# raguilar011095/planet_heightmap_generation

Hardware: AMD Instinct MI355X
Metric: Mcells·iter/s, terrain-post erosion stack (higher is better)
Workload: dtype f64

## Files before the change

planet_heightmap_generation_amd/csrc/basin.hip:

```cpp
#include <hip/hip_runtime.h>

#include <string>

#include "device.h"

namespace wo {

namespace {

constexpr int32_t WO_RANGE_NONE = 0x7f7f7f7f;
#ifndef WO_BASIN_RANGE_SLOTS
#define WO_BASIN_RANGE_SLOTS 256
#endif
constexpr int WO_BASIN_RANGE = WO_BASIN_RANGE_SLOTS;
constexpr int WO_BASIN_KEY_BITS = 16;
constexpr int WO_BASIN_CHASE_CAP = 1 << 16;

__device__ inline int32_t basin_root(int32_t* J, int32_t s) {
    auto ld = [&](int32_t x) { return __atomic_load_n(&J[x], __ATOMIC_RELAXED); };
    int32_t j = ld(s), tort = j;
    int power = 1, lam = 0;
    for (int it = 0; it < WO_BASIN_CHASE_CAP; ++it) {
        const int32_t jj = ld(j);
        if (jj == j) return j;
        if (jj == tort) {
            int32_t m = jj, y = ld(jj);
            for (int k = 0; k < WO_BASIN_CHASE_CAP && y != jj; ++k) {
                const int32_t yy = ld(y);
                if (yy == y) return y;
                m = y < m ? y : m;
                y = yy;
            }
            __atomic_store_n(&J[m], m, __ATOMIC_RELAXED);
            return m;
        }
        if (++lam == power) { tort = jj; power <<= 1; lam = 0; }
        j = jj;
    }
    return j;
}

__global__ __launch_bounds__(WO_BLOCK) void k_basin_jump(const int32_t* __restrict__ slotCell, int32_t* J, int32_t L, int32_t shift, uint32_t* __restrict__ keyOfCell) {
    for (int32_t s = blockIdx.x * blockDim.x + threadIdx.x; s < L; s += gridDim.x * blockDim.x) {
        const int32_t j = basin_root(J, s);
        __atomic_store_n(&J[s], j, __ATOMIC_RELAXED);
        keyOfCell[slotCell ? slotCell[s] : s] = (uint32_t)j >> shift;
    }
}
__global__ __launch_bounds__(WO_BLOCK) void k_basin_keys(const int32_t* __restrict__ land, const uint32_t* __restrict__ keyOfCell, int32_t L,
                                                          uint32_t* __restrict__ keys, int32_t* __restrict__ vals, int32_t scramble, int32_t* rangeStart, int32_t nRangeWords) {
    for (int32_t i = blockIdx.x * blockDim.x + threadIdx.x; i < nRangeWords; i += gridDim.x * blockDim.x) rangeStart[i] = WO_RANGE_NONE;
    if (blockIdx.x == 0 && threadIdx.x == 0) rangeStart[nRangeWords] = 0;
    for (int32_t i = blockIdx.x * blockDim.x + threadIdx.x; i < L; i += gridDim.x * blockDim.x) {
        const int32_t c = land[L - 1 - i];
        keys[i] = (scramble && c % 3 == 0) ? (keyOfCell[c] ^ 1u) : keyOfCell[c];
        vals[i] = c;
    }
}

__global__ __launch_bounds__(WO_BLOCK) void k_basin_slots(const int32_t* __restrict__ order, const uint32_t* __restrict__ keys, int32_t* __restrict__ slotOf, int32_t L,
                                                           int32_t* rangeStart, int32_t rangeT) {
    for (int32_t q = blockIdx.x * blockDim.x + threadIdx.x; q < L; q += gridDim.x * blockDim.x) {
        if (slotOf) slotOf[order[q]] = q;
        if (q == 0 || keys[q] != keys[q - 1]) atomicMin(&rangeStart[q / rangeT], q);
    }
}

#ifndef WO_LONG_RANGE_SLOTS
#define WO_LONG_RANGE_SLOTS 2048
#endif
#ifndef WO_LONG_LIST
#define WO_LONG_LIST 2048
#endif
constexpr int32_t WO_LONG_RANGE = WO_LONG_RANGE_SLOTS, WO_LONG_MAX = WO_LONG_LIST;
__device__ inline int32_t range_end(const int32_t* __restrict__ rangeStart, int32_t k, int32_t nRanges, int32_t L) {
    for (int32_t j = k + 1; j < nRanges; ++j) { const int32_t v = rangeStart[j]; if (v != WO_RANGE_NONE) return v; }
    return L;
}
__global__ __launch_bounds__(WO_BLOCK) void k_basin_long(const int32_t* __restrict__ rangeStart, int32_t nRanges, int32_t L, int32_t* big, uint8_t* __restrict__ flag) {
    for (int32_t k = blockIdx.x * blockDim.x + threadIdx.x; k < nRanges; k += gridDim.x * blockDim.x) {
        const int32_t S = rangeStart[k];
        uint8_t f = 0;
        if (S != WO_RANGE_NONE && range_end(rangeStart, k, nRanges, L) - S >= WO_LONG_RANGE) {
            const int32_t at = atomicAdd(&big[0], 1);
            if (at < WO_LONG_MAX) { big[1 + at] = k; f = 1; }
        }
        flag[k] = f;
    }
}
__device__ inline bool block_range(const int32_t* __restrict__ rangeStart, int32_t nRanges, int32_t L, const int32_t* __restrict__ big, const uint8_t* __restrict__ flag, int32_t& S, int32_t& E) {
    int32_t k;
    if (big) {
        if ((int32_t)blockIdx.x < WO_LONG_MAX) { const int32_t n = big[0] < WO_LONG_MAX ? big[0] : WO_LONG_MAX; if ((int32_t)blockIdx.x >= n) return false; k = big[1 + blockIdx.x]; }
        else { k = (int32_t)blockIdx.x - WO_LONG_MAX; if (flag[k]) return false; }
    } else k = (int32_t)blockIdx.x;
    S = rangeStart[k];
    if (S == WO_RANGE_NONE) return false;
    E = range_end(rangeStart, k, nRanges, L);
// ... 174 lines not shown
        if (lane == 0) { s_passes[wave] = myPasses; s_readyPasses[wave] = myReady; }
        if (tid == 0) { s_clk[0] = cWait; s_clk[1] = cTurn; s_clk[2] = myPasses; s_clk[3] = cRest; }
        __syncthreads();
        if (tid == 0) {
            const unsigned long long c = (unsigned long long)(clock64() - cStart);
            const unsigned long long packed = (c << 24) | (unsigned long long)(s_maxLevel & 0xffffff);
            const unsigned long long old = atomicMax(&stats[0], packed);
            if (packed > old) {
                stats[1] = (unsigned long long)(E - S);
                unsigned long long mp = 0, mr = 0;
                for (int w = 0; w < NW; ++w) { mp = s_passes[w] > mp ? s_passes[w] : mp; mr = s_readyPasses[w] > mr ? s_readyPasses[w] : mr; }
                stats[2] = mp; stats[3] = mr; stats[4] = s_clk[0]; stats[5] = s_clk[1]; stats[6] = s_clk[2]; stats[7] = s_clk[3];
            }
        }
    }
}

}

void basin_alloc(wo_planet* p) {
    const int32_t N = p->N;
    hipStream_t s = cur_stream(p);
    if (!p->d_basinJ) {
        WO_HIP(hipMalloc((void**)&p->d_basinJ, (size_t)N * 4));
        WO_HIP(hipMalloc((void**)&p->d_basinSlot, (size_t)N * 4));
        WO_HIP(hipMalloc((void**)&p->d_basinKey, (size_t)N * 4));
        WO_HIP(hipMalloc((void**)&p->d_basinVals[0], (size_t)N * 4)); WO_HIP(hipMalloc((void**)&p->d_basinVals[1], (size_t)N * 4));
        WO_HIP(hipMalloc((void**)&p->d_basinRange, ((size_t)N / 64 + 8 + WO_LONG_MAX) * 4));
        WO_HIP(hipMalloc((void**)&p->d_basinLong, (size_t)N / 64 + 8));
        WO_HIP(hipMemsetAsync(p->d_basinSlot, 0xff, (size_t)N * 4, s));
    }
}

void basin_layout(wo_planet* p, bool slotIdentity) {
    const int32_t L = p->L;
    basin_alloc(p);
    int bitsL = 1;
    while (((int64_t)1 << bitsL) < (int64_t)L) ++bitsL;
    const int shift = bitsL > WO_BASIN_KEY_BITS ? bitsL - WO_BASIN_KEY_BITS : 0;
    const int grid = blocks_for(L, 1 << 16);
    launch(p, FAM_BASIN, k_basin_jump, grid, WO_BLOCK, slotIdentity ? (const int32_t*)nullptr : (const int32_t*)p->d_patchOrder, p->d_basinJ, L, (int32_t)shift, p->d_basinKey);
    const int rangeT = WO_BASIN_RANGE;
    const int nRanges = (int)(((int64_t)L + rangeT - 1) / rangeT);
    launch(p, FAM_BASIN, k_basin_keys, grid, WO_BLOCK, (const int32_t*)p->d_land[p->landCur], (const uint32_t*)p->d_basinKey, L, p->d_keys[0], p->d_basinVals[0],
           (int32_t)(p->opt.basinScramble ? 1 : 0), p->d_basinRange, (int32_t)(nRanges + 1));
    uint32_t* const kb[2] = {p->d_keys[0], p->d_keys[1]};
    int32_t* const vb[2] = {p->d_basinVals[0], p->d_basinVals[1]};
    const int sorted = radix_sort_pairs(p, FAM_BASIN_SORT, kb, vb, L, 0, 16 , p->d_basinSlot, radix_scratch(p, 1), p->N, p->rsFlip[1]);
    launch(p, FAM_BASIN, k_basin_slots, blocks_for(L, 4096), WO_BLOCK, (const int32_t*)p->d_basinVals[sorted], (const uint32_t*)p->d_keys[sorted], (int32_t*)nullptr, L, p->d_basinRange, (int32_t)rangeT);
    launch(p, FAM_BASIN, k_basin_long, blocks_for(nRanges), WO_BLOCK, (const int32_t*)p->d_basinRange, (int32_t)nRanges, L, p->d_basinRange + nRanges + 1, p->d_basinLong);
}

void basin_solve_launch(wo_planet* p, const Fields& F, int32_t launchTag, int32_t* totalPending) {
    const int nRanges = (int)(((int64_t)p->L + WO_BASIN_RANGE - 1) / WO_BASIN_RANGE);
    ++p->basinLaunches;
    const int32_t* big = (const int32_t*)(p->d_basinRange + nRanges + 1);
    const uint8_t* flag = (const uint8_t*)p->d_basinLong;
    const int grid = nRanges + WO_LONG_MAX;
    launch(p, FAM_SOLVE_BASIN, k_solve_flowing<2, false>, grid, 128, F, p->L, (const int32_t*)p->d_basinRange, (int32_t)nRanges, launchTag, p->d_patchPending, totalPending, big, flag, (unsigned long long*)nullptr);
}

void basin_free(wo_planet* p) {
    if (p->d_basinJ) (void)hipFree(p->d_basinJ);
    if (p->d_basinSlot) (void)hipFree(p->d_basinSlot);
    if (p->d_basinKey) (void)hipFree(p->d_basinKey);
    for (auto& v : p->d_basinVals) { if (v) (void)hipFree(v); v = nullptr; }
    if (p->d_basinRange) (void)hipFree(p->d_basinRange);
    if (p->d_basinLong) (void)hipFree(p->d_basinLong);
    p->d_basinLong = nullptr;
    p->d_basinJ = nullptr; p->d_basinSlot = nullptr; p->d_basinKey = nullptr; p->d_basinRange = nullptr;
}

}
```

planet_heightmap_generation_amd/csrc/device.h:

```cpp
#pragma once
#include <hip/hip_runtime.h>

#include <cstdint>
#include <cstdio>
#include <map>
#include <string>
#include <vector>

#include "host_util.h"

#include "erode_ops.h"
#include "flood_ops.h"
#include "wo_internal.h"

namespace wo {

struct HipError { std::string msg; };

#define WO_HIP(call)                                                                                   \
    do {                                                                                               \
        hipError_t e_ = (call);                                                                        \
        if (e_ != hipSuccess)                                                                          \
            throw ::wo::HipError{std::string(#call) + " -> " + hipGetErrorString(e_) + " (" + __FILE__ + ":" + \
                                 std::to_string(__LINE__) + ")"};                                      \
// ... 82 lines not shown
    wo::FloodExchange floodX;
    void* floodLink = nullptr; void (*floodLinkFree)(void*) = nullptr;
    wo_flood_gpu fgpu;

    int32_t *d_off = nullptr, *d_adj = nullptr;
    float *d_dist = nullptr, *d_xyz = nullptr;
    float *d_e = nullptr, *d_e2 = nullptr, *d_hot = nullptr, *d_orig = nullptr;
    uint8_t *d_ocean = nullptr, *d_coast = nullptr;
    int64_t mirrorMaskVersion = -1;
    uint8_t* d_oceanKnown = nullptr; int32_t* d_maskDiff = nullptr; bool oceanKnownValid = false;
    bool hot_valid = false;
    float* d_savedE = nullptr; uint8_t* d_savedOcean = nullptr; bool saved = false;
    uint8_t* d_tables = nullptr;
    bool scratch = false;
    bool landIdentity = false;
    int64_t floodPrefixMirror = -1, floodPrefixStatic = -1;
    bool floodPrefixOk = false;
    int32_t *d_landIdx = nullptr, *d_land[2] = {nullptr, nullptr}, *d_rank = nullptr;
    int32_t* d_landInit = nullptr; int64_t oceanVersion = 0, landListsOcean = -1; bool landListsMirror = false; int32_t landListsL = -1;
    uint32_t* d_keys[2] = {nullptr, nullptr};
    float *d_cellDist = nullptr, *d_flow = nullptr;
    wo::SolveTask* d_task = nullptr; wo::SolveOut* d_out = nullptr; int32_t *d_haloSend = nullptr, *d_haloRecv = nullptr; float *d_haloBuf = nullptr, *h_haloBuf = nullptr; int32_t nHaloSend = 0, nHaloRecv = 0;
    int32_t* d_flowCnt = nullptr; wo::TargetRank* d_tr = nullptr; wo::EventList* d_ev = nullptr; float* d_me = nullptr;
    int32_t *d_carveSlot = nullptr, *d_carveDeps = nullptr, *d_carveDepCnt = nullptr, *d_carveDepPos = nullptr; uint32_t* d_rs[2] = {nullptr, nullptr}; int rsFlip[2] = {0, 0};    wo::CarveRec* d_carveRecs = nullptr; wo::CarveExpect* d_carveExpect = nullptr; unsigned long long* d_carveG = nullptr;    int32_t* d_carveSlotDone = nullptr; int64_t carveCap = 0;
    unsigned long long* d_accCnt = nullptr;
    int32_t *d_ftLr = nullptr, *d_ftParent = nullptr, *d_ftExtCnt = nullptr; uint32_t* d_ftInflow = nullptr; unsigned long long* d_ftRootAcc = nullptr;
    int32_t *d_jump = nullptr, *d_nj = nullptr;
    int32_t* d_doneAt = nullptr;
    double* d_totalExcess = nullptr;
    float *d_glac = nullptr, *d_iceFlow = nullptr;
    int32_t *d_iceTarget = nullptr, *d_arank = nullptr;
    uint8_t* d_iceUp = nullptr;
    int32_t *d_patchOrder = nullptr, *d_slotOf = nullptr, *d_patchPending = nullptr, *d_patchTotals = nullptr, *d_patchBlk = nullptr; int64_t patchVersion = -1; bool patchMirror = false; int32_t numPatches = 0; int64_t lastPatchLaunches = 1; int64_t solveCalls = 0;
    hipStream_t side = nullptr; hipEvent_t evFork = nullptr, evJoin = nullptr; bool onSide = false;
    uint32_t* d_basinKey = nullptr; int32_t* d_basinVals[2] = {nullptr, nullptr}; int32_t *d_basinJ = nullptr, *d_basinSlot = nullptr, *d_basinRange = nullptr; uint8_t* d_basinLong = nullptr; int64_t basinLaunches = 0; wo::Affine* d_affine[2] = {nullptr, nullptr};    int64_t solvePassSerial = 0;
    int32_t* h_patchTotals = nullptr;
    int32_t *d_listA = nullptr, *d_listB = nullptr, *d_counters = nullptr;
    void* d_sortTemp = nullptr; size_t sortTempBytes = 0;
    int landCur = 0;
    int32_t L = 0;

    struct Import {
        uint8_t* img = nullptr; int64_t imgCap = 0;
        int32_t* label = nullptr;
        uint8_t* flags = nullptr;
        int32_t* lists = nullptr;
        uint8_t* seedOcean = nullptr;
        int32_t* blockCounts = nullptr;
        int32_t* totals = nullptr; int32_t* h_totals = nullptr;
    } imp;

    struct wo_wind_block* wind = nullptr;
    struct wo_ocean_block* ocean = nullptr;

    struct Mirror {
        bool built = false, active = false;
        int32_t *perm = nullptr, *inv = nullptr, *off = nullptr, *adj = nullptr;
        float *dist = nullptr, *xyz = nullptr, *e = nullptr, *e2 = nullptr, *hot = nullptr;
        uint8_t *ocean = nullptr, *coast = nullptr;
        wo::hvec<int32_t> h_perm, h_morton;
        wo::hvec<uint8_t> h_mask;
        int64_t version = 0;
        int32_t *o_off = nullptr, *o_adj = nullptr; float *o_dist = nullptr, *o_xyz = nullptr, *o_e = nullptr, *o_e2 = nullptr;
        uint8_t *o_ocean = nullptr, *o_coast = nullptr;
    } mirror;

    hipEvent_t evStart = nullptr, evStop = nullptr;
// ... 20 lines not shown

template <class... KArgs, class... Args>
inline void launch(wo_planet* p, int fam, void (*kernel)(KArgs...), int grid, int block, Args... args) {
    hipStream_t s = cur_stream(p);
    if (p->profiling) {
        hipEvent_t a = profile_event(p), b = profile_event(p);
        WO_HIP(hipEventRecord(a, s));
        hipLaunchKernelGGL(kernel, dim3(grid), dim3(block), 0, s, args...);
        WO_HIP(hipGetLastError());
        WO_HIP(hipEventRecord(b, s));
        p->pending.push_back({fam, a, b});
        if (p->pending.size() >= 4096) profile_resolve(p);
    } else {
        hipLaunchKernelGGL(kernel, dim3(grid), dim3(block), 0, s, args...);
        WO_HIP(hipGetLastError());
    }
}

template <class... KArgs, class... Args>
inline void launch_shmem(wo_planet* p, int fam, void (*kernel)(KArgs...), int grid, int block, size_t shmem, Args... args) {
    hipStream_t s = p->ctx->stream;
    hipEvent_t a = nullptr, b = nullptr;
    if (p->profiling) { a = profile_event(p); b = profile_event(p); WO_HIP(hipEventRecord(a, s)); }
    if (shmem > (size_t)(64 << 10)) WO_HIP(hipFuncSetAttribute(reinterpret_cast<const void*>(kernel), hipFuncAttributeMaxDynamicSharedMemorySize, (int)shmem));
    hipLaunchKernelGGL(kernel, dim3(grid), dim3(block), shmem, s, args...);
    WO_HIP(hipGetLastError());
    if (p->profiling) { WO_HIP(hipEventRecord(b, s)); p->pending.push_back({fam, a, b}); if (p->pending.size() >= 4096) profile_resolve(p); }
}

void sort_land_by_elevation(wo_planet* p);
size_t sort_temp_bytes(int32_t n);
void rank_from_land(wo_planet* p);
size_t radix_scratch_words(int32_t nMax);
int radix_sort_pairs(wo_planet* p, int family, uint32_t* const keys[2], int32_t* const vals[2], int32_t n, int beginBit, int endBit, int32_t* posOut,
                     uint32_t* scratch, int32_t nMax, int& flip);
uint32_t* radix_scratch(wo_planet* p, int which);
void select_active_by_rank(wo_planet* p, const int32_t* arank, int32_t* out, int32_t* outCount);
void basin_alloc(wo_planet* p);
void basin_layout(wo_planet* p, bool slotIdentity);
void basin_solve_launch(wo_planet* p, const Fields& F, int32_t launchTag, int32_t* totalPending);
void basin_free(wo_planet* p);
void import_free(wo_planet* p);
void wind_free(wo_planet* p);
void ocean_free(wo_planet* p);
bool check_planet(wo_planet* p, const char* fn);
float* smooth_field_resident(wo_planet* p, float* a, float* b, int32_t passes);

}
```

planet_heightmap_generation_amd/csrc/planet.hip:

```cpp
#include <hip/hip_runtime.h>

#include <algorithm>
#include <atomic>
#include <chrono>
#include <cmath>
#include <cstring>

#include "../../include/worogen.h"
#include "device.h"
#include "elevation_host.h"
#include "elevation_kernels.h"
#include "kernels_impl.h"
#include "flood_kernels.h"
#include "elevation_bfs.h"
#include "noise.h"

namespace wo {

const char* const kFamilyNames[FAM_COUNT] = {
    "coast_flags", "smooth_elevation", "sharpen_ridges", "soil_creep", "warp_terrain", "noise_eval", "synthetic_terrain",
    "ocean_from_elevation", "sort_keys", "sort_radix", "rank_scatter", "receivers", "flow_climb",
    "flow_final", "solve_setup", "solve_round", "solve_final", "thermal_excess", "thermal_apply",
    "glac_index", "ice_receivers", "ice_round", "carve_setup", "carve_round", "moraine_fjord", "glacial_blend", "solve_patch", "elev_collisions", "elev_uplift_fused", "plate_grid", "plate_project", "smooth_field", "flood_eval", "flood_apply", "flood_misc", "climate_sweeps", "basin_layout", "basin_sort", "solve_basin", "flow_tiles", "misc", "event_pair_empty", "event_pair_noop_kernel", "event_pair_two_noop_kernels"};

// ... 458 lines not shown
        const int32_t N = p->N;
        launch(p, FAM_MISC, k_mirror_gather_f32, blocks_for(N, 4096), WO_BLOCK, (const float*)p->d_e, (const int32_t*)M.perm, M.e, N);
        launch(p, FAM_MISC, k_mirror_gather_u8, blocks_for(N, 4096), WO_BLOCK, (const uint8_t*)p->d_ocean, (const int32_t*)M.perm, M.ocean, N);
        M.o_off = p->d_off; M.o_adj = p->d_adj; M.o_dist = p->d_dist; M.o_xyz = p->d_xyz; M.o_e = p->d_e; M.o_e2 = p->d_e2; M.o_ocean = p->d_ocean; M.o_coast = p->d_coast;
        point_at_mirror(M.e, M.e2);
        M.active = on = true;
    }
    void suspend() {
        if (!on) return;
        auto& M = p->mirror;
        launch(p, FAM_MISC, k_mirror_scatter_f32, blocks_for(p->N, 4096), WO_BLOCK, (const float*)p->d_e, (const int32_t*)M.perm, M.o_e, p->N);
        cur = p->d_e; cur2 = p->d_e2;
        point_at_planet();
    }
    void resume() {
        if (!on) return;
        auto& M = p->mirror;
        launch(p, FAM_MISC, k_mirror_gather_f32, blocks_for(p->N, 4096), WO_BLOCK, (const float*)M.o_e, (const int32_t*)M.perm, cur, p->N);
        point_at_mirror(cur, cur2);
    }
    void finish() {
        if (!on) return;
        suspend();
        p->mirror.active = on = false;
    }
    ~MirrorScope() { if (on) { point_at_planet(); p->mirror.active = false; } }
};

static void ensure_side_stream(wo_planet* p) {
    if (p->side) return;
    int prLeast = 0, prGreatest = 0;
    WO_HIP(hipDeviceGetStreamPriorityRange(&prLeast, &prGreatest));
    WO_HIP(hipStreamCreateWithPriority(&p->side, hipStreamNonBlocking, prGreatest));
    WO_HIP(hipEventCreateWithFlags(&p->evFork, hipEventDisableTiming)); WO_HIP(hipEventCreateWithFlags(&p->evJoin, hipEventDisableTiming));
}

struct RedoWithChecks {};

struct ErodeCall {
    wo_planet* p;
    int32_t hIters; double K, m, dt; int32_t tIters; double talus, kThermal; int32_t gIters; double gStrength; bool checkEveryPass;
    int32_t total, midIter; double gCarve, gConv, gDep, gFjord;
    int gridN, gridL = 0;
    StageClock clk; MirrorScope mir; FloodRun floodRun;
    int64_t sorts = 0, maxSolve = 0, patchLaunches = 0, basinPasses = 0, basinLeftoverPasses = 0, iceRounds = 0, carveRounds = 0, carveActive = 0, carveFlowLeft = 0;
    double floodHostMs = 0;
    ErodeCall(wo_planet* pl, int32_t h, double K_, double m_, double dt_, int32_t t, double talus_, double kT, int32_t g, double gs, bool check)
        : p(pl), hIters(h), K(K_), m(m_), dt(dt_), tIters(t), talus(talus_), kThermal(kT), gIters(std::max(g, 0)), gStrength(gs != gs ? 0 : gs),
          checkEveryPass(check), total(std::max(hIters, std::max(tIters, gIters))), midIter((int32_t)std::floor(total * 0.75 + 0.5)),
          gridN(xcd_grid(pl->N)), clk(pl), mir(pl) {
        const double gScale = gIters > 0 ? 1.0 / gIters : 0;
        gCarve = 0.02 * gScale; gConv = 0.01 * gScale; gDep = 0.005 * gScale; gFjord = 0.015 * gScale;
    }
    void stats(bool mirrored) const {
        p->erodeStats = {{"land_cells", (double)p->L}, {"mirror_layout", mirrored ? 1.0 : 0.0}, {"iterations", (double)total}, {"sorts", (double)sorts},
                         {"solve_launches_max_per_pass", (double)maxSolve}, {"solve_patch_launches_total", (double)patchLaunches},
                         {"solve_basin_passes", (double)basinPasses}, {"solve_basin_passes_with_leftovers", (double)basinLeftoverPasses},
                         {"flow_two_level", (p->d_ftLr && p->landIdentity && hIters > 0) ? 1.0 : 0.0}, {"ice_rounds_total", (double)iceRounds},
                         {"carve_rounds_total", (double)carveRounds}, {"carve_active_total", (double)carveActive}, {"carve_flow_launches_with_leftovers", (double)carveFlowLeft}, {"solve_check_every_pass", checkEveryPass ? 1.0 : 0.0}, {"calls_run_again_with_checks", (double)p->redoCalls}, {"flood_stage_ms", floodHostMs},
                         {"flood_device_pass1_ms", floodRun.deviceMs}, {"flood_device_rounds", (double)floodRun.rounds}, {"flood_device_epochs", (double)floodRun.epochs},
                         {"flood_device_evaluations", (double)floodRun.evals}, {"flood_equal_key_decisions", (double)floodRun.ties}, {"flood_pass1_on_host", (floodRun.usedDevice && !floodRun.fellBack) ? 0.0 : 1.0},
                         {"flood_host_calls", (double)floodRun.host.calls}, {"flood_host_serial_pass1", (double)floodRun.host.serialPass1}, {"flood_host_tie_groups", (double)floodRun.host.tieGroups}, {"flood_host_contested", (double)floodRun.host.contested},
                         {"flood_host_open_parents", (double)floodRun.host.openParents}, {"flood_host_unresolved", (double)floodRun.host.unresolved},
                         {"flood_host_path_redo", (double)floodRun.host.pathRedo}, {"flood_host_replays", (double)floodRun.host.replays}, {"flood_host_replayed_landmasses", (double)floodRun.host.replayedLandmasses}, {"flood_host_pass1_ms", floodRun.host.pass1Ms},
                         {"flood_host_pass23_ms", floodRun.host.pass23Ms},
                         {"relaxed_sort_every", (double)p->opt.relaxedSortEvery}, {"relaxed_full", p->opt.relaxedFull ? 1.0 : 0.0}, {"flood_exchange_calls", (double)p->floodX.calls}, {"flood_exchange_gathers", (double)p->floodX.gathers}, {"flood_exchange_whole_planet_floods", (double)p->floodX.globalFloods}, {"flood_exchange_received", (double)p->floodX.received}};
    }
// ... 165 lines not shown
    c.clk.begin("glacial");
    Fields F = p->fields();
    ice_flow(c, F);
    launch(p, FAM_CARVE_SETUP, k_carve_setup_cells, c.gridN, WO_BLOCK, F);
    select_active_by_rank(p, F.arank, p->d_listB, p->d_counters + 3);
    const int32_t active = read_count(p, p->d_counters + 3);
    c.carveActive += active; ensure_carve_capacity(p, active);
    F.carveDeps = p->d_carveDeps; F.carveDepCnt = p->d_carveDepCnt; F.carveDepPos = p->d_carveDepPos;
    if (active > 0) c.carveRounds += carve_launches(c, F, active);
    launch(p, FAM_MORAINE, k_moraine_fjord, c.gridN, WO_BLOCK, F, c.gDep, c.gFjord);
    c.clk.end();
}
static FlowTiles flow_tiles_buffers(wo_planet* p) {
    const size_t N = (size_t)p->N;
    if (!p->d_ftLr) {
        p->d_ftLr = dalloc<int32_t>(N); p->d_ftParent = dalloc<int32_t>(N); p->d_ftExtCnt = dalloc<int32_t>(N); p->d_ftInflow = dalloc<uint32_t>(N); p->d_ftRootAcc = dalloc<unsigned long long>(N);
        WO_HIP(hipMemsetAsync(p->d_ftInflow, 0, N * 4, p->ctx->stream)); WO_HIP(hipMemsetAsync(p->d_ftExtCnt, 0, N * 4, p->ctx->stream));
    }
    FlowTiles FT{};
    FT.lr = p->d_ftLr; FT.parent = p->d_ftParent; FT.rootAcc = p->d_ftRootAcc; FT.inflow = p->d_ftInflow; FT.extCnt = p->d_ftExtCnt;
    return FT;
}
static int flow_tile_count(int32_t L) { return (int)(((int64_t)L + FT_CELLS - 1) / FT_CELLS); }
static void erode_receivers(ErodeCall& c, const Fields& F, const FlowTiles& FT, int32_t* donorCnt, bool basin, bool slotIdentity, bool tilesBeforeFork) {
    wo_planet* p = c.p; hipStream_t s = p->ctx->stream;
    Fields Fr = F; if (basin) Fr.basinJ = p->d_basinJ;
    c.clk.begin("receivers");
    launch(p, FAM_RECEIVERS, k_receivers_flow_init, c.gridL, WO_BLOCK, Fr, donorCnt);
    c.clk.end();
    if (!basin) return;
    ensure_side_stream(p);
    if (tilesBeforeFork) {
        launch(p, FAM_FLOW_TILES, k_flow_tiles<false>, flow_tile_count(p->L), FT_THREADS, F, FT);
        launch(p, FAM_FLOW_TILES, k_flow_root_links, blocks_for(p->L, 4096), WO_BLOCK, F, FT);
    }
    WO_HIP(hipEventRecord(p->evFork, s));
    WO_HIP(hipStreamWaitEvent(p->side, p->evFork, 0));
    p->onSide = true;
    try { basin_layout(p, slotIdentity); } catch (...) { p->onSide = false; throw; }
    p->onSide = false;
    WO_HIP(hipEventRecord(p->evJoin, p->side));
}
static void erode_flow(ErodeCall& c, const Fields& F, const FlowTiles& FT, int32_t* donorCnt, bool flowTiles, bool tilesBeforeFork, bool clearOut) {
    wo_planet* p = c.p;
    c.clk.begin("flow");
    if (flowTiles) {
        const int tiles = flow_tile_count(p->L);
        if (!tilesBeforeFork) {
            launch(p, FAM_FLOW_TILES, k_flow_tiles<false>, tiles, FT_THREADS, F, FT);
            launch(p, FAM_FLOW_TILES, k_flow_root_links, blocks_for(p->L, 4096), WO_BLOCK, F, FT);
        }
        launch(p, FAM_FLOW_TILES, k_flow_root_climb, blocks_for(p->L, 4096), WO_BLOCK, F, FT);
        launch(p, FAM_FLOW_TILES, k_flow_tiles<true>, tiles, FT_THREADS, F, FT);
    } else
        launch(p, FAM_FLOW_SNAP, k_flow_climb, c.gridL, WO_BLOCK, F, (const int32_t*)p->d_flowCnt, (int32_t)0x7fffffff);
    Fields Ff = F;
    if (p->opt.relaxedFull) Ff.ev = nullptr;
    launch(p, FAM_FLOW_FINAL, k_flow_final, c.gridL, WO_BLOCK, Ff, donorCnt, clearOut ? p->d_out : (SolveOut*)nullptr);
    c.clk.end();
}
static void erode_solve_basin(ErodeCall& c, Fields F, int32_t iter) {
    wo_planet* p = c.p; hipStream_t s = p->ctx->stream;
    WO_HIP(hipStreamWaitEvent(s, p->evJoin, 0));
    F.slotOf = p->d_basinSlot; F.solveLean = 1;
    const bool unchecked = !c.checkEveryPass; F.solveFinals = unchecked ? 1 : 0;
    launch(p, FAM_SOLVE_SETUP, k_solve_setup_batched<true>, c.gridL, WO_BLOCK, F, p->d_patchPending, (int32_t)p->numPatches, p->d_patchTotals, (int32_t)WO_PATCH_TOTAL_SLOTS);
    int32_t passTag = 1;
    if (unchecked) {
        if (p->solvePassSerial >= 0x3ff00000) { WO_HIP(hipMemsetAsync(p->d_out, 0, (size_t)p->N * sizeof(SolveOut), s)); p->solvePassSerial = 0; }
        passTag = (1 << 20) + (int32_t)(++p->solvePassSerial);
    }
    const int64_t r = run_solve_patches(p, F, c.K, c.m, c.dt, unchecked, passTag);
    ++c.basinPasses; if (r > 1) ++c.basinLeftoverPasses;
    c.patchLaunches += r; c.maxSolve = std::max(c.maxSolve, r);
    if (!unchecked) launch(p, FAM_SOLVE_FINAL, k_solve_final, c.gridL, WO_BLOCK, F, p->d_e2, (iter < c.tIters) ? p->d_me : (float*)nullptr);
}
static void erode_solve_affine(ErodeCall& c, const Fields& F) {
    wo_planet* p = c.p;
    if (!p->d_affine[0]) { p->d_affine[0] = dalloc<Affine>((size_t)p->N); p->d_affine[1] = dalloc<Affine>((size_t)p->N); }
    launch(p, FAM_SOLVE_SETUP, k_affine_init, c.gridL, WO_BLOCK, F, p->d_affine[0]);
    int cur = 0;
    for (int q = 0; q < 12; ++q, cur ^= 1) launch(p, FAM_SOLVE_ROUND, k_affine_jump, c.gridL, WO_BLOCK, F, (const Affine*)p->d_affine[cur], p->d_affine[cur ^ 1]);
    launch(p, FAM_SOLVE_FINAL, k_affine_apply, c.gridL, WO_BLOCK, F, (const Affine*)p->d_affine[cur], p->d_e2);
}
static void hydraulic_step(ErodeCall& c, int32_t iter) {
    wo_planet* p = c.p;
    Fields F = p->fields();
    F.solveK = c.K; F.solveM = c.m; F.solveDt = c.dt;
    const bool basin = !p->opt.relaxedFull;
    const bool slotIdentity = c.mir.on && p->mirror.h_mask.size() == (size_t)p->N;
    if (basin) { basin_alloc(p); F.basinMslot = slotIdentity ? nullptr : p->d_slotOf; }
    const bool flowTiles = p->landIdentity;
    FlowTiles FT = flowTiles ? flow_tiles_buffers(p) : FlowTiles{};
    const bool tilesBeforeFork = basin && flowTiles && slotIdentity;
    if (tilesBeforeFork) FT.basinJ = p->d_basinJ;
    int32_t* const donorCnt = flowTiles ? (int32_t*)nullptr : p->d_flowCnt;
    erode_receivers(c, F, FT, donorCnt, basin, slotIdentity, tilesBeforeFork);
    erode_flow(c, F, FT, donorCnt, flowTiles, tilesBeforeFork, basin && c.checkEveryPass);
    c.clk.begin("solve");
    if (basin) erode_solve_basin(c, F, iter); else erode_solve_affine(c, F);
    swap_elev(p);
    c.clk.end();
}
static void thermal_step(ErodeCall& c, bool afterSolve) {
// ... 257 lines not shown
            WO_HIP(hipMemcpyAsync(p->d_dist, neighborDist, (size_t)E * 4, hipMemcpyHostToDevice, s));
        } else {
            std::vector<float> nd(E);
            neighbor_dist(N, adjOffset, adjList, r_xyz, nd.data());
            WO_HIP(hipMemcpyAsync(p->d_dist, nd.data(), (size_t)E * 4, hipMemcpyHostToDevice, s));
            WO_HIP(hipStreamSynchronize(s));
        }
        WO_HIP(hipMemsetAsync(p->d_e, 0, (size_t)N * 4, s));
        WO_HIP(hipMemsetAsync(p->d_ocean, 0, (size_t)N, s));
        WO_HIP(hipEventCreate(&p->evStart)); WO_HIP(hipEventCreate(&p->evStop));
        WO_HIP(hipStreamSynchronize(s));
        return p;
    } catch (const HipError& e) {
        set_error(std::string("wo_planet_create: ") + e.msg);
        if (p) wo_planet_destroy(p);
        return nullptr;
    }
}

void wo_planet_destroy(wo_planet* p) {
    if (!p) return;
    (void)hipSetDevice(p->ctx->device);
    (void)hipStreamSynchronize(p->ctx->stream);
    dfree(p->d_off); dfree(p->d_adj); dfree(p->d_dist); dfree(p->d_xyz); dfree(p->d_e); dfree(p->d_e2); dfree(p->d_hot); dfree(p->d_orig);
    flood_gpu_free(p->fgpu);
    if (p->floodLink && p->floodLinkFree) p->floodLinkFree(p->floodLink);
    p->floodLink = nullptr;
    basin_free(p);
    import_free(p);
    ocean_free(p);
    wind_free(p);
    if (p->side) { (void)hipStreamSynchronize(p->side); (void)hipStreamDestroy(p->side); p->side = nullptr; }
    if (p->evFork) { (void)hipEventDestroy(p->evFork); p->evFork = nullptr; }
    if (p->evJoin) { (void)hipEventDestroy(p->evJoin); p->evJoin = nullptr; }
    mirror_free(p);
    dfree(p->d_ocean); dfree(p->d_coast); dfree(p->d_tables); dfree(p->d_savedE); dfree(p->d_savedOcean);
    if (p->d_oceanKnown) { (void)hipFree(p->d_oceanKnown); p->d_oceanKnown = nullptr; } if (p->d_maskDiff) { (void)hipFree(p->d_maskDiff); p->d_maskDiff = nullptr; }
    dfree(p->d_landInit); dfree(p->d_landIdx); dfree(p->d_land[0]); dfree(p->d_land[1]); dfree(p->d_keys[0]); dfree(p->d_keys[1]); dfree(p->d_rank);
    dfree(p->d_cellDist); dfree(p->d_flow); dfree(p->d_task); dfree(p->d_out); dfree(p->d_flowCnt); dfree(p->d_tr); dfree(p->d_ev); dfree(p->d_me); dfree(p->d_haloSend); dfree(p->d_haloRecv); dfree(p->d_haloBuf); if (p->h_haloBuf) { (void)hipHostFree(p->h_haloBuf); p->h_haloBuf = nullptr; } dfree(p->d_carveSlot); dfree(p->d_redoE); dfree(p->d_pendingEver); for (auto& r : p->d_rs) { if (r) (void)hipFree(r); r = nullptr; } dfree(p->d_carveG); dfree(p->d_carveExpect); dfree(p->d_carveRecs); dfree(p->d_carveSlotDone); dfree(p->d_carveDeps); dfree(p->d_carveDepCnt); dfree(p->d_carveDepPos); dfree(p->d_ftLr); dfree(p->d_ftParent); dfree(p->d_affine[0]); dfree(p->d_affine[1]); dfree(p->d_ftExtCnt); dfree(p->d_ftInflow); dfree(p->d_ftRootAcc); dfree(p->d_accCnt); dfree(p->d_jump); dfree(p->d_nj);
    dfree(p->d_doneAt); dfree(p->d_totalExcess);
    dfree(p->d_glac); dfree(p->d_iceFlow); dfree(p->d_iceTarget); dfree(p->d_arank); dfree(p->d_iceUp);
    dfree(p->d_patchOrder); dfree(p->d_slotOf); dfree(p->d_patchPending); dfree(p->d_patchTotals); dfree(p->d_patchBlk);
    dfree(p->d_listA); dfree(p->d_listB); dfree(p->d_counters);
    if (p->h_patchTotals) (void)hipHostFree(p->h_patchTotals);
    if (p->d_sortTemp) (void)hipFree(p->d_sortTemp);
    if (p->h_pinned) (void)hipHostFree(p->h_pinned);
    if (p->h_count) (void)hipHostFree(p->h_count);
    if (p->h_word) { (void)hipHostFree(p->h_word); p->h_word = nullptr; }
    for (auto& pe : p->pending) { (void)hipEventDestroy(pe.a); (void)hipEventDestroy(pe.b); }
    for (auto& b : p->stageBrackets) { (void)hipEventDestroy(b.a); (void)hipEventDestroy(b.b); }
    for (auto e : p->eventPool) (void)hipEventDestroy(e);
    if (p->evStart) (void)hipEventDestroy(p->evStart);
    if (p->evStop) (void)hipEventDestroy(p->evStop);
    delete p;
}

int wo_planet_upload(wo_planet* p, const float* r_elevation, const uint8_t* r_isOcean) {
    if (!check_planet(p, "wo_planet_upload")) return 1;
    WO_TRY
    hipStream_t s = p->ctx->stream;
    if (r_elevation) WO_HIP(hipMemcpyAsync(p->d_e, r_elevation, (size_t)p->N * 4, hipMemcpyHostToDevice, s));
    if (r_isOcean) {
        WO_HIP(hipMemcpyAsync(p->d_ocean, r_isOcean, (size_t)p->N, hipMemcpyHostToDevice, s));
        if (p->h_ocean.size() != (size_t)p->N || std::memcmp(p->h_ocean.data(), r_isOcean, (size_t)p->N) != 0) {
            p->h_ocean.assign(r_isOcean, r_isOcean + p->N);
            p->flood.staticValid = false; ++p->oceanVersion;
// ... 677 lines not shown
```

planet_heightmap_generation_amd/csrc/radix.hip:

```cpp
#include <hip/hip_runtime.h>

#include <cstdint>
#include <cstdlib>

#include "device.h"

namespace wo {

namespace {
#ifndef WO_RS_ITEMS
#define WO_RS_ITEMS 16
#endif
constexpr int RS_THREADS = 256, RS_WAVES = 4, RS_ITEMS = WO_RS_ITEMS, RS_TILE = RS_THREADS * RS_ITEMS, RS_DIGITS = 256;

constexpr int RS_GROUP = 32;

__global__ __launch_bounds__(RS_THREADS) void k_rs_count(const uint32_t* __restrict__ keys, int32_t n, int shift, uint32_t* __restrict__ counts, uint32_t* groupTot) {
    __shared__ uint32_t s_c[RS_WAVES][RS_DIGITS];
    const int lane = threadIdx.x & 63, wave = threadIdx.x >> 6;
#pragma unroll
    for (int w = 0; w < RS_WAVES; ++w) s_c[w][threadIdx.x] = 0;
    const int32_t tile = blockIdx.x;
    const int32_t first = tile * RS_TILE + wave * (64 * RS_ITEMS) + lane;
    uint32_t key[RS_ITEMS];
#pragma unroll
    for (int j = 0; j < RS_ITEMS; ++j) { const int32_t i = first + j * 64; key[j] = i < n ? keys[i] : 0u; }
    __syncthreads();
#pragma unroll
    for (int j = 0; j < RS_ITEMS; ++j) if (first + j * 64 < n) atomicAdd(&s_c[wave][(key[j] >> shift) & 255u], 1u);
    __syncthreads();
    const uint32_t c = s_c[0][threadIdx.x] + s_c[1][threadIdx.x] + s_c[2][threadIdx.x] + s_c[3][threadIdx.x];
    counts[(size_t)tile * RS_DIGITS + threadIdx.x] = c;
    if (c) atomicAdd(&groupTot[(size_t)(tile / RS_GROUP) * RS_DIGITS + threadIdx.x], c);
}

__global__ __launch_bounds__(RS_THREADS) void k_rs_scatter(const uint32_t* __restrict__ keysIn, const int32_t* __restrict__ valsIn, uint32_t* __restrict__ keysOut,
                                                          int32_t* __restrict__ valsOut, int32_t n, int shift, const uint32_t* __restrict__ counts,
                                                          const uint32_t* __restrict__ groupTot, int32_t groups, uint32_t* clearNext, int32_t* __restrict__ posOut) {
    __shared__ uint32_t s_cnt[RS_WAVES][RS_DIGITS];
    __shared__ uint32_t s_off[RS_DIGITS];
    __shared__ uint32_t s_start[RS_DIGITS];
    __shared__ uint32_t s_wsum[2][RS_WAVES];
    __shared__ uint32_t s_keys[RS_TILE];
    __shared__ int32_t s_vals[RS_TILE];
    const int lane = threadIdx.x & 63, wave = threadIdx.x >> 6;
    const int32_t tile = blockIdx.x;
    const int32_t tileFirst = tile * RS_TILE;
    const int32_t first = tileFirst + wave * (64 * RS_ITEMS) + lane;
    uint32_t key[RS_ITEMS]; int32_t val[RS_ITEMS]; uint32_t rnk[RS_ITEMS];
#pragma unroll
    for (int j = 0; j < RS_ITEMS; ++j) {
        const int32_t i = first + j * 64;
        const bool ok = i < n;
        key[j] = ok ? keysIn[i] : 0xffffffffu;
        val[j] = ok ? valsIn[i] : 0;
    }
    uint32_t excl = 0, histD = 0;
    {
        const int d = threadIdx.x;
        const int32_t g = tile / RS_GROUP;
        uint32_t v[16];
        for (int32_t q0 = 0; q0 < groups; q0 += 16) {
#pragma unroll
            for (int u = 0; u < 16; ++u) v[u] = (q0 + u < groups) ? groupTot[(size_t)(q0 + u) * RS_DIGITS + d] : 0u;
#pragma unroll
            for (int u = 0; u < 16; ++u) { histD += v[u]; if (q0 + u < g) excl += v[u]; }
        }
#pragma unroll
// ... 42 lines not shown
        for (int w = 0; w < RS_WAVES; ++w) { c[w] = s_cnt[w][d]; }
#pragma unroll
        for (int w = 0; w < RS_WAVES; ++w) { s_cnt[w][d] = total; total += c[w]; }
        uint32_t incl = total;
#pragma unroll
        for (int o = 1; o < 64; o <<= 1) { const uint32_t t = __shfl_up(incl, o); if (lane >= o) incl += t; }
        if (lane == 63) s_wsum[1][wave] = incl;
        __syncthreads();
        uint32_t before = 0;
#pragma unroll
        for (int w = 0; w < RS_WAVES; ++w) if (w < wave) before += s_wsum[1][w];
        const uint32_t start = before + incl - total;
        s_start[d] = start;
        s_off[d] = hbase + excl - start;
    }
    __syncthreads();
#pragma unroll
    for (int j = 0; j < RS_ITEMS; ++j) {
        if (first + j * 64 >= n) continue;
        const uint32_t d = (key[j] >> shift) & 255u;
        const uint32_t q = s_start[d] + s_cnt[wave][d] + rnk[j];
        s_keys[q] = key[j];
        s_vals[q] = val[j];
    }
    __syncthreads();
    const int32_t have = min((int32_t)RS_TILE, n - tileFirst);
#pragma unroll
    for (int j = 0; j < RS_ITEMS; ++j) {
        const int32_t q = j * RS_THREADS + (int32_t)threadIdx.x;
        if (q >= have) continue;
        const uint32_t k = s_keys[q];
        const int32_t v = s_vals[q];
        const uint32_t dst = s_off[(k >> shift) & 255u] + (uint32_t)q;
        keysOut[dst] = k;
        valsOut[dst] = v;
        if (posOut) posOut[v] = (int32_t)dst;
    }
}
}

static inline int rs_tiles(int32_t n) { return (int)(((int64_t)n + RS_TILE - 1) / RS_TILE); }

static inline int rs_groups(int32_t n) { return (rs_tiles(n) + RS_GROUP - 1) / RS_GROUP; }
size_t radix_scratch_words(int32_t nMax) { return (size_t)2 * rs_groups(nMax) * RS_DIGITS + (size_t)rs_tiles(nMax) * RS_DIGITS; }

int radix_sort_pairs(wo_planet* p, int family, uint32_t* const keys[2], int32_t* const vals[2], int32_t n, int beginBit, int endBit, int32_t* posOut,
                     uint32_t* scratch, int32_t nMax, int& flip) {
    const int passes = (endBit - beginBit + 7) / 8;
    if (passes <= 0 || n <= 0) return 0;
    if (passes & 1) throw HipError{"radix_sort_pairs: the number of digits must be even"};
    if (n > nMax) throw HipError{"radix_sort_pairs: more pairs than the scratch was sized for"};
    hipStream_t s = cur_stream(p);
    const int tiles = rs_tiles(n), groups = rs_groups(n);
    const size_t gtWords = (size_t)rs_groups(nMax) * RS_DIGITS;
    uint32_t* counts = scratch + 2 * gtWords;
    auto bracketed = [&](auto&& launchIt) {
        hipEvent_t a = nullptr, b = nullptr;
        if (p->profiling) { a = profile_event(p); b = profile_event(p); WO_HIP(hipEventRecord(a, s)); }
        launchIt();
        if (p->profiling) { WO_HIP(hipEventRecord(b, s)); p->pending.push_back({family, a, b}); if (p->pending.size() >= 4096) profile_resolve(p); }
    };
    int cur = 0;
    for (int q = 0; q < passes; ++q, ++flip) {
        uint32_t* gt = scratch + (size_t)(flip & 1) * gtWords;
        uint32_t* gtOther = scratch + (size_t)((flip + 1) & 1) * gtWords;
        bracketed([&] { hipLaunchKernelGGL(k_rs_count, dim3(tiles), dim3(RS_THREADS), 0, s, (const uint32_t*)keys[cur], n, beginBit + 8 * q, counts, gt); });
        bracketed([&] { hipLaunchKernelGGL(k_rs_scatter, dim3(tiles), dim3(RS_THREADS), 0, s, (const uint32_t*)keys[cur], (const int32_t*)vals[cur], keys[cur ^ 1], vals[cur ^ 1], n,
                           beginBit + 8 * q, (const uint32_t*)counts, (const uint32_t*)gt, (int32_t)groups, gtOther, (q == passes - 1) ? posOut : (int32_t*)nullptr); });
        cur ^= 1;
    }
    WO_HIP(hipGetLastError());
    return cur;
}

uint32_t* radix_scratch(wo_planet* p, int which) {
    if (!p->d_rs[which]) {
        const size_t words = radix_scratch_words(p->N);
        WO_HIP(hipMalloc((void**)&p->d_rs[which], words * 4));
        WO_HIP(hipMemsetAsync(p->d_rs[which], 0, words * 4, cur_stream(p)));
        p->rsFlip[which] = 0;
    }
    return p->d_rs[which];
}

}
```

planet_heightmap_generation_amd/csrc/sort.hip:

```cpp
#include <hip/hip_runtime.h>

#include <algorithm>
#include <cstdio>
#include <string>
#include <cstdlib>

#include "device.h"

namespace wo {

__global__ __launch_bounds__(WO_BLOCK) void k_sort_keys(const float* __restrict__ e, const int32_t* __restrict__ land,
                                                         uint32_t* __restrict__ keys, int32_t L) {
    for (int32_t i = blockIdx.x * blockDim.x + threadIdx.x; i < L; i += gridDim.x * blockDim.x)
        keys[i] = desc_key(e[land[i]]);
}

__global__ __launch_bounds__(WO_BLOCK) void k_rank_scatter(const int32_t* __restrict__ land, int32_t* __restrict__ rank, int32_t L) {
    for (int32_t i = blockIdx.x * blockDim.x + threadIdx.x; i < L; i += gridDim.x * blockDim.x)
        rank[land[i]] = i;
}

void rank_from_land(wo_planet* p) {
    launch(p, FAM_RANK, k_rank_scatter, blocks_for(p->L, 4096), WO_BLOCK, (const int32_t*)p->d_land[p->landCur], p->d_rank, p->L);
}
// ... 36 lines not shown
    }
    if (threadIdx.x == 0) *outCount = run;
}
__global__ __launch_bounds__(WO_BLOCK) void k_sel_scatter(const int32_t* __restrict__ land, const int32_t* __restrict__ arank, int32_t L, const int32_t* __restrict__ tileStart, int32_t* __restrict__ out) {
    __shared__ int32_t s_wave[WO_BLOCK / 64];
    const int32_t base = blockIdx.x * WO_SEL_TILE + threadIdx.x * WO_SEL_PER_THREAD;
    int32_t cell[WO_SEL_PER_THREAD]; bool on[WO_SEL_PER_THREAD];
    int32_t c = 0;
#pragma unroll
    for (int q = 0; q < WO_SEL_PER_THREAD; ++q) { const int32_t i = base + q; cell[q] = i < L ? land[i] : 0; on[q] = i < L && arank[cell[q]] != WO_NOT_DONE; c += on[q] ? 1 : 0; }
    int32_t total;
    int32_t at = tileStart[blockIdx.x] + block_exclusive_scan(c, s_wave, total);
#pragma unroll
    for (int q = 0; q < WO_SEL_PER_THREAD; ++q) if (on[q]) out[at++] = cell[q];
}
void select_active_by_rank(wo_planet* p, const int32_t* arank, int32_t* out, int32_t* outCount) {
    const int32_t L = p->L;
    const int nTiles = (int)(((int64_t)L + WO_SEL_TILE - 1) / WO_SEL_TILE);
    int32_t* tileCnt = reinterpret_cast<int32_t*>(p->d_sortTemp);
    const int32_t* land = p->d_land[p->landCur];
    launch(p, FAM_CARVE_SETUP, k_sel_count, nTiles, WO_BLOCK, land, arank, L, tileCnt);
    launch(p, FAM_CARVE_SETUP, k_sel_scan, 1, WO_BLOCK, tileCnt, (int32_t)nTiles, outCount);
    launch(p, FAM_CARVE_SETUP, k_sel_scatter, nTiles, WO_BLOCK, land, arank, L, (const int32_t*)tileCnt, out);
}

size_t sort_temp_bytes(int32_t n) { return ((size_t)n / WO_SEL_TILE + 2) * sizeof(int32_t); }

void sort_land_by_elevation(wo_planet* p) {
    const int32_t L = p->L;
    const int cur = p->landCur;
    launch(p, FAM_SORT_KEYS, k_sort_keys, blocks_for(L, 4096), WO_BLOCK, (const float*)p->d_e, (const int32_t*)p->d_land[cur], p->d_keys[0], L);
    uint32_t* const kb[2] = {p->d_keys[0], p->d_keys[1]};
    int32_t* const vb[2] = {p->d_land[cur], p->d_land[cur ^ 1]};
    const int r = radix_sort_pairs(p, FAM_SORT_RADIX, kb, vb, L, 0, 32, p->d_rank, radix_scratch(p, 0), p->N, p->rsFlip[0]);
    p->landCur = r == 0 ? cur : (cur ^ 1);
}

}
```

Measured before the change: 6399.

## Split basin layout to overlap solve setup and skip unused radix outputs

Basin layout is split into a slot phase (jump, keys, sort) and a ranges phase, with a new event so the main stream's solve setup can start once slots are ready and only wait for the range tables before the patch solve. The root-links kernel moves after the fork so it overlaps with the side-stream basin work. The radix sort gains a template option to skip writing keys or values on the last pass: the basin sort writes only keys and the elevation sort only values. In slot-identity mode the key lookup reads roots directly instead of writing an intermediate key array. This adds another event and more cross-stream ordering to get right.

```diff
diff --git a/planet_heightmap_generation_amd/csrc/basin.hip b/planet_heightmap_generation_amd/csrc/basin.hip
--- a/planet_heightmap_generation_amd/csrc/basin.hip
+++ b/planet_heightmap_generation_amd/csrc/basin.hip
@@ -44,26 +44,24 @@
     for (int32_t s = blockIdx.x * blockDim.x + threadIdx.x; s < L; s += gridDim.x * blockDim.x) {
         const int32_t j = basin_root(J, s);
         __atomic_store_n(&J[s], j, __ATOMIC_RELAXED);
-        keyOfCell[slotCell ? slotCell[s] : s] = (uint32_t)j >> shift;
-    }
-}
-__global__ __launch_bounds__(WO_BLOCK) void k_basin_keys(const int32_t* __restrict__ land, const uint32_t* __restrict__ keyOfCell, int32_t L,
+        if (slotCell) keyOfCell[slotCell[s]] = (uint32_t)j >> shift;
+    }
+}
+__global__ __launch_bounds__(WO_BLOCK) void k_basin_keys(const int32_t* __restrict__ land, const uint32_t* __restrict__ keyOfCell, const int32_t* __restrict__ rootOf, int32_t shift, int32_t L,
                                                           uint32_t* __restrict__ keys, int32_t* __restrict__ vals, int32_t scramble, int32_t* rangeStart, int32_t nRangeWords) {
     for (int32_t i = blockIdx.x * blockDim.x + threadIdx.x; i < nRangeWords; i += gridDim.x * blockDim.x) rangeStart[i] = WO_RANGE_NONE;
     if (blockIdx.x == 0 && threadIdx.x == 0) rangeStart[nRangeWords] = 0;
     for (int32_t i = blockIdx.x * blockDim.x + threadIdx.x; i < L; i += gridDim.x * blockDim.x) {
         const int32_t c = land[L - 1 - i];
-        keys[i] = (scramble && c % 3 == 0) ? (keyOfCell[c] ^ 1u) : keyOfCell[c];
+        const uint32_t k = keyOfCell ? keyOfCell[c] : ((uint32_t)rootOf[c] >> shift);
+        keys[i] = (scramble && c % 3 == 0) ? (k ^ 1u) : k;
         vals[i] = c;
     }
 }
 
-__global__ __launch_bounds__(WO_BLOCK) void k_basin_slots(const int32_t* __restrict__ order, const uint32_t* __restrict__ keys, int32_t* __restrict__ slotOf, int32_t L,
-                                                           int32_t* rangeStart, int32_t rangeT) {
-    for (int32_t q = blockIdx.x * blockDim.x + threadIdx.x; q < L; q += gridDim.x * blockDim.x) {
-        if (slotOf) slotOf[order[q]] = q;
+__global__ __launch_bounds__(WO_BLOCK) void k_basin_slots(const uint32_t* __restrict__ keys, int32_t L, int32_t* rangeStart, int32_t rangeT) {
+    for (int32_t q = blockIdx.x * blockDim.x + threadIdx.x; q < L; q += gridDim.x * blockDim.x)
         if (q == 0 || keys[q] != keys[q - 1]) atomicMin(&rangeStart[q / rangeT], q);
-    }
 }
 
 #ifndef WO_LONG_RANGE_SLOTS
@@ -304,7 +302,7 @@
     }
 }
 
-void basin_layout(wo_planet* p, bool slotIdentity) {
+int basin_layout_slots(wo_planet* p, bool slotIdentity) {
     const int32_t L = p->L;
     basin_alloc(p);
     int bitsL = 1;
@@ -312,14 +310,18 @@
     const int shift = bitsL > WO_BASIN_KEY_BITS ? bitsL - WO_BASIN_KEY_BITS : 0;
     const int grid = blocks_for(L, 1 << 16);
     launch(p, FAM_BASIN, k_basin_jump, grid, WO_BLOCK, slotIdentity ? (const int32_t*)nullptr : (const int32_t*)p->d_patchOrder, p->d_basinJ, L, (int32_t)shift, p->d_basinKey);
+    const int nRanges = (int)(((int64_t)L + WO_BASIN_RANGE - 1) / WO_BASIN_RANGE);
+    launch(p, FAM_BASIN, k_basin_keys, grid, WO_BLOCK, (const int32_t*)p->d_land[p->landCur], slotIdentity ? (const uint32_t*)nullptr : (const uint32_t*)p->d_basinKey,
+           (const int32_t*)p->d_basinJ, (int32_t)shift, L, p->d_keys[0], p->d_basinVals[0], (int32_t)(p->opt.basinScramble ? 1 : 0), p->d_basinRange, (int32_t)(nRanges + 1));
+    uint32_t* const kb[2] = {p->d_keys[0], p->d_keys[1]};
+    int32_t* const vb[2] = {p->d_basinVals[0], p->d_basinVals[1]};
+    return radix_sort_pairs(p, FAM_BASIN_SORT, kb, vb, L, 0, 16 , p->d_basinSlot, radix_scratch(p, 1), p->N, p->rsFlip[1], RS_OUT_KEYS);
+}
+void basin_layout_ranges(wo_planet* p, int sortedKeys) {
+    const int32_t L = p->L;
     const int rangeT = WO_BASIN_RANGE;
     const int nRanges = (int)(((int64_t)L + rangeT - 1) / rangeT);
-    launch(p, FAM_BASIN, k_basin_keys, grid, WO_BLOCK, (const int32_t*)p->d_land[p->landCur], (const uint32_t*)p->d_basinKey, L, p->d_keys[0], p->d_basinVals[0],
-           (int32_t)(p->opt.basinScramble ? 1 : 0), p->d_basinRange, (int32_t)(nRanges + 1));
-    uint32_t* const kb[2] = {p->d_keys[0], p->d_keys[1]};
-    int32_t* const vb[2] = {p->d_basinVals[0], p->d_basinVals[1]};
-    const int sorted = radix_sort_pairs(p, FAM_BASIN_SORT, kb, vb, L, 0, 16 , p->d_basinSlot, radix_scratch(p, 1), p->N, p->rsFlip[1]);
-    launch(p, FAM_BASIN, k_basin_slots, blocks_for(L, 4096), WO_BLOCK, (const int32_t*)p->d_basinVals[sorted], (const uint32_t*)p->d_keys[sorted], (int32_t*)nullptr, L, p->d_basinRange, (int32_t)rangeT);
+    launch(p, FAM_BASIN, k_basin_slots, blocks_for(L, 4096), WO_BLOCK, (const uint32_t*)p->d_keys[sortedKeys], L, p->d_basinRange, (int32_t)rangeT);
     launch(p, FAM_BASIN, k_basin_long, blocks_for(nRanges), WO_BLOCK, (const int32_t*)p->d_basinRange, (int32_t)nRanges, L, p->d_basinRange + nRanges + 1, p->d_basinLong);
 }
 
diff --git a/planet_heightmap_generation_amd/csrc/device.h b/planet_heightmap_generation_amd/csrc/device.h
--- a/planet_heightmap_generation_amd/csrc/device.h
+++ b/planet_heightmap_generation_amd/csrc/device.h
@@ -138,7 +138,7 @@
     int32_t *d_iceTarget = nullptr, *d_arank = nullptr;
     uint8_t* d_iceUp = nullptr;
     int32_t *d_patchOrder = nullptr, *d_slotOf = nullptr, *d_patchPending = nullptr, *d_patchTotals = nullptr, *d_patchBlk = nullptr; int64_t patchVersion = -1; bool patchMirror = false; int32_t numPatches = 0; int64_t lastPatchLaunches = 1; int64_t solveCalls = 0;
-    hipStream_t side = nullptr; hipEvent_t evFork = nullptr, evJoin = nullptr; bool onSide = false;
+    hipStream_t side = nullptr; hipEvent_t evFork = nullptr, evSlots = nullptr, evJoin = nullptr; bool onSide = false;
     uint32_t* d_basinKey = nullptr; int32_t* d_basinVals[2] = {nullptr, nullptr}; int32_t *d_basinJ = nullptr, *d_basinSlot = nullptr, *d_basinRange = nullptr; uint8_t* d_basinLong = nullptr; int64_t basinLaunches = 0; wo::Affine* d_affine[2] = {nullptr, nullptr};    int64_t solvePassSerial = 0;
     int32_t* h_patchTotals = nullptr;
     int32_t *d_listA = nullptr, *d_listB = nullptr, *d_counters = nullptr;
@@ -225,12 +225,14 @@
 size_t sort_temp_bytes(int32_t n);
 void rank_from_land(wo_planet* p);
 size_t radix_scratch_words(int32_t nMax);
+enum { RS_OUT_KEYS = 1, RS_OUT_VALS = 2, RS_OUT_BOTH = 3 };
 int radix_sort_pairs(wo_planet* p, int family, uint32_t* const keys[2], int32_t* const vals[2], int32_t n, int beginBit, int endBit, int32_t* posOut,
-                     uint32_t* scratch, int32_t nMax, int& flip);
+                     uint32_t* scratch, int32_t nMax, int& flip, int lastOut = RS_OUT_BOTH);
 uint32_t* radix_scratch(wo_planet* p, int which);
 void select_active_by_rank(wo_planet* p, const int32_t* arank, int32_t* out, int32_t* outCount);
 void basin_alloc(wo_planet* p);
-void basin_layout(wo_planet* p, bool slotIdentity);
+int basin_layout_slots(wo_planet* p, bool slotIdentity);
+void basin_layout_ranges(wo_planet* p, int sortedKeys);
 void basin_solve_launch(wo_planet* p, const Fields& F, int32_t launchTag, int32_t* totalPending);
 void basin_free(wo_planet* p);
 void import_free(wo_planet* p);
diff --git a/planet_heightmap_generation_amd/csrc/planet.hip b/planet_heightmap_generation_amd/csrc/planet.hip
--- a/planet_heightmap_generation_amd/csrc/planet.hip
+++ b/planet_heightmap_generation_amd/csrc/planet.hip
@@ -514,7 +514,7 @@
     int prLeast = 0, prGreatest = 0;
     WO_HIP(hipDeviceGetStreamPriorityRange(&prLeast, &prGreatest));
     WO_HIP(hipStreamCreateWithPriority(&p->side, hipStreamNonBlocking, prGreatest));
-    WO_HIP(hipEventCreateWithFlags(&p->evFork, hipEventDisableTiming)); WO_HIP(hipEventCreateWithFlags(&p->evJoin, hipEventDisableTiming));
+    WO_HIP(hipEventCreateWithFlags(&p->evFork, hipEventDisableTiming)); WO_HIP(hipEventCreateWithFlags(&p->evSlots, hipEventDisableTiming)); WO_HIP(hipEventCreateWithFlags(&p->evJoin, hipEventDisableTiming));
 }
 
 struct RedoWithChecks {};
@@ -746,12 +746,16 @@
     ensure_side_stream(p);
     if (tilesBeforeFork) {
         launch(p, FAM_FLOW_TILES, k_flow_tiles<false>, flow_tile_count(p->L), FT_THREADS, F, FT);
-        launch(p, FAM_FLOW_TILES, k_flow_root_links, blocks_for(p->L, 4096), WO_BLOCK, F, FT);
     }
     WO_HIP(hipEventRecord(p->evFork, s));
     WO_HIP(hipStreamWaitEvent(p->side, p->evFork, 0));
+    if (tilesBeforeFork) launch(p, FAM_FLOW_TILES, k_flow_root_links, blocks_for(p->L, 4096), WO_BLOCK, F, FT);
     p->onSide = true;
-    try { basin_layout(p, slotIdentity); } catch (...) { p->onSide = false; throw; }
+    try {
+        const int sortedKeys = basin_layout_slots(p, slotIdentity);
+        WO_HIP(hipEventRecord(p->evSlots, p->side));
+        basin_layout_ranges(p, sortedKeys);
+    } catch (...) { p->onSide = false; throw; }
     p->onSide = false;
     WO_HIP(hipEventRecord(p->evJoin, p->side));
 }
@@ -775,7 +779,7 @@
 }
 static void erode_solve_basin(ErodeCall& c, Fields F, int32_t iter) {
     wo_planet* p = c.p; hipStream_t s = p->ctx->stream;
-    WO_HIP(hipStreamWaitEvent(s, p->evJoin, 0));
+    WO_HIP(hipStreamWaitEvent(s, p->evSlots, 0));
     F.slotOf = p->d_basinSlot; F.solveLean = 1;
     const bool unchecked = !c.checkEveryPass; F.solveFinals = unchecked ? 1 : 0;
     launch(p, FAM_SOLVE_SETUP, k_solve_setup_batched<true>, c.gridL, WO_BLOCK, F, p->d_patchPending, (int32_t)p->numPatches, p->d_patchTotals, (int32_t)WO_PATCH_TOTAL_SLOTS);
@@ -784,6 +788,7 @@
         if (p->solvePassSerial >= 0x3ff00000) { WO_HIP(hipMemsetAsync(p->d_out, 0, (size_t)p->N * sizeof(SolveOut), s)); p->solvePassSerial = 0; }
         passTag = (1 << 20) + (int32_t)(++p->solvePassSerial);
     }
+    WO_HIP(hipStreamWaitEvent(s, p->evJoin, 0));
     const int64_t r = run_solve_patches(p, F, c.K, c.m, c.dt, unchecked, passTag);
     ++c.basinPasses; if (r > 1) ++c.basinLeftoverPasses;
     c.patchLaunches += r; c.maxSolve = std::max(c.maxSolve, r);
@@ -1107,6 +1112,7 @@
     wind_free(p);
     if (p->side) { (void)hipStreamSynchronize(p->side); (void)hipStreamDestroy(p->side); p->side = nullptr; }
     if (p->evFork) { (void)hipEventDestroy(p->evFork); p->evFork = nullptr; }
+    if (p->evSlots) { (void)hipEventDestroy(p->evSlots); p->evSlots = nullptr; }
     if (p->evJoin) { (void)hipEventDestroy(p->evJoin); p->evJoin = nullptr; }
     mirror_free(p);
     dfree(p->d_ocean); dfree(p->d_coast); dfree(p->d_tables); dfree(p->d_savedE); dfree(p->d_savedOcean);
diff --git a/planet_heightmap_generation_amd/csrc/radix.hip b/planet_heightmap_generation_amd/csrc/radix.hip
--- a/planet_heightmap_generation_amd/csrc/radix.hip
+++ b/planet_heightmap_generation_amd/csrc/radix.hip
@@ -34,6 +34,7 @@
     if (c) atomicAdd(&groupTot[(size_t)(tile / RS_GROUP) * RS_DIGITS + threadIdx.x], c);
 }
 
+template <bool KEYS_OUT, bool VALS_OUT>
 __global__ __launch_bounds__(RS_THREADS) void k_rs_scatter(const uint32_t* __restrict__ keysIn, const int32_t* __restrict__ valsIn, uint32_t* __restrict__ keysOut,
                                                           int32_t* __restrict__ valsOut, int32_t n, int shift, const uint32_t* __restrict__ counts,
                                                           const uint32_t* __restrict__ groupTot, int32_t groups, uint32_t* clearNext, int32_t* __restrict__ posOut) {
@@ -142,8 +143,8 @@
         const uint32_t k = s_keys[q];
         const int32_t v = s_vals[q];
         const uint32_t dst = s_off[(k >> shift) & 255u] + (uint32_t)q;
-        keysOut[dst] = k;
-        valsOut[dst] = v;
+        if (KEYS_OUT) keysOut[dst] = k;
+        if (VALS_OUT) valsOut[dst] = v;
         if (posOut) posOut[v] = (int32_t)dst;
     }
 }
@@ -155,11 +156,12 @@
 size_t radix_scratch_words(int32_t nMax) { return (size_t)2 * rs_groups(nMax) * RS_DIGITS + (size_t)rs_tiles(nMax) * RS_DIGITS; }
 
 int radix_sort_pairs(wo_planet* p, int family, uint32_t* const keys[2], int32_t* const vals[2], int32_t n, int beginBit, int endBit, int32_t* posOut,
-                     uint32_t* scratch, int32_t nMax, int& flip) {
+                     uint32_t* scratch, int32_t nMax, int& flip, int lastOut) {
     const int passes = (endBit - beginBit + 7) / 8;
     if (passes <= 0 || n <= 0) return 0;
     if (passes & 1) throw HipError{"radix_sort_pairs: the number of digits must be even"};
     if (n > nMax) throw HipError{"radix_sort_pairs: more pairs than the scratch was sized for"};
+    if ((lastOut & RS_OUT_BOTH) == 0) throw HipError{"radix_sort_pairs: the last pass must write the keys or the values"};
     hipStream_t s = cur_stream(p);
     const int tiles = rs_tiles(n), groups = rs_groups(n);
     const size_t gtWords = (size_t)rs_groups(nMax) * RS_DIGITS;
@@ -175,8 +177,12 @@
         uint32_t* gt = scratch + (size_t)(flip & 1) * gtWords;
         uint32_t* gtOther = scratch + (size_t)((flip + 1) & 1) * gtWords;
         bracketed([&] { hipLaunchKernelGGL(k_rs_count, dim3(tiles), dim3(RS_THREADS), 0, s, (const uint32_t*)keys[cur], n, beginBit + 8 * q, counts, gt); });
-        bracketed([&] { hipLaunchKernelGGL(k_rs_scatter, dim3(tiles), dim3(RS_THREADS), 0, s, (const uint32_t*)keys[cur], (const int32_t*)vals[cur], keys[cur ^ 1], vals[cur ^ 1], n,
-                           beginBit + 8 * q, (const uint32_t*)counts, (const uint32_t*)gt, (int32_t)groups, gtOther, (q == passes - 1) ? posOut : (int32_t*)nullptr); });
+        const bool last = q == passes - 1;
+        auto* scatter = k_rs_scatter<true, true>;
+        if (last && (lastOut & RS_OUT_BOTH) == RS_OUT_KEYS) scatter = k_rs_scatter<true, false>;
+        if (last && (lastOut & RS_OUT_BOTH) == RS_OUT_VALS) scatter = k_rs_scatter<false, true>;
+        bracketed([&] { hipLaunchKernelGGL(scatter, dim3(tiles), dim3(RS_THREADS), 0, s, (const uint32_t*)keys[cur], (const int32_t*)vals[cur], keys[cur ^ 1], vals[cur ^ 1], n,
+                           beginBit + 8 * q, (const uint32_t*)counts, (const uint32_t*)gt, (int32_t)groups, gtOther, last ? posOut : (int32_t*)nullptr); });
         cur ^= 1;
     }
     WO_HIP(hipGetLastError());
diff --git a/planet_heightmap_generation_amd/csrc/sort.hip b/planet_heightmap_generation_amd/csrc/sort.hip
--- a/planet_heightmap_generation_amd/csrc/sort.hip
+++ b/planet_heightmap_generation_amd/csrc/sort.hip
@@ -92,7 +92,7 @@
     launch(p, FAM_SORT_KEYS, k_sort_keys, blocks_for(L, 4096), WO_BLOCK, (const float*)p->d_e, (const int32_t*)p->d_land[cur], p->d_keys[0], L);
     uint32_t* const kb[2] = {p->d_keys[0], p->d_keys[1]};
     int32_t* const vb[2] = {p->d_land[cur], p->d_land[cur ^ 1]};
-    const int r = radix_sort_pairs(p, FAM_SORT_RADIX, kb, vb, L, 0, 32, p->d_rank, radix_scratch(p, 0), p->N, p->rsFlip[0]);
+    const int r = radix_sort_pairs(p, FAM_SORT_RADIX, kb, vb, L, 0, 32, p->d_rank, radix_scratch(p, 0), p->N, p->rsFlip[0], RS_OUT_VALS);
     p->landCur = r == 0 ? cur : (cur ^ 1);
 }
 
```

Result: no change. 6344 (-0.9%).
